# entn-at/tf-kaldi-speaker

Hardware: AMD Instinct MI355X
Metric: utterances/sec x-vector extraction (30-dim x 300-frame) (higher is better)
Workload: dtype f16+fp6-cross(f32-split); 1 GPU; tdnn x-vector (tdnn6_dense), statistics_pooling, 256 utt/GPU/step of 300 frames x 30 dims; batch_per_gpu=256, frames=300, node=tdnn6_dense, precision=f16f6, parallelism=utterance-shard x1, launch=stream launches

## Files before the change

### tf-kaldi-speaker_amd/csrc/gemm_f32.hip

```cpp
#include <mutex>

#include "xv_epilogue.h"

namespace xv {

constexpr int BM = 128, BN = 128, BK = 32;
constexpr int LDT = BK + 4;
constexpr int TILE_F = BM * LDT;

template <int FORM>
__global__ __launch_bounds__(256, 2) void gemm_f32_kernel(GemmArgs p, int nMt, int nNt, int kper) {
  extern __shared__ __attribute__((aligned(16))) float smem[];
  float* As = smem;
  float* Bs = smem + 2 * TILE_F;

  const int tid = threadIdx.x;
  const int lane = tid & 63, wave = tid >> 6;
  const int wm = wave >> 1, wn = wave & 1;
  const int r32 = lane & 31, h = lane >> 5;

  const int ntiles = nMt * nNt;
  const int slice = blockIdx.x / ntiles;
  const int tile = xcd_remap(blockIdx.x - slice * ntiles, ntiles);
  const int mt = tile / nNt, nt = tile - mt * nNt;
// ... 80 lines not shown
    for (int q = 0; q < BK / 8; ++q) {
      f32x4 a0 = *reinterpret_cast<const f32x4*>(ap + q * 8);
      f32x4 a1 = *reinterpret_cast<const f32x4*>(ap + 32 * LDT + q * 8);
      f32x4 b0 = *reinterpret_cast<const f32x4*>(bp + q * 8);
      f32x4 b1 = *reinterpret_cast<const f32x4*>(bp + 32 * LDT + q * 8);
#pragma unroll
      for (int j = 0; j < 4; ++j) {
        acc[0][0] = __builtin_amdgcn_mfma_f32_32x32x2f32(b0[j], a0[j], acc[0][0], 0, 0, 0);
        acc[0][1] = __builtin_amdgcn_mfma_f32_32x32x2f32(b0[j], a1[j], acc[0][1], 0, 0, 0);
        acc[1][0] = __builtin_amdgcn_mfma_f32_32x32x2f32(b1[j], a0[j], acc[1][0], 0, 0, 0);
        acc[1][1] = __builtin_amdgcn_mfma_f32_32x32x2f32(b1[j], a1[j], acc[1][1], 0, 0, 0);
      }
    }
    if (kt + 1 < nk) store_tiles(cur ^ 1);
    __syncthreads();
  }

  store_wave_tile(p, acc, m0 + wm * 64, n0 + wn * 64, lane, wave, reinterpret_cast<char*>(smem));
}

__global__ void splitk_reduce_kernel(GemmArgs p) {
  const int64_t total = (int64_t)p.M * p.N;
  for (int64_t i = (int64_t)blockIdx.x * blockDim.x + threadIdx.x; i < total; i += (int64_t)gridDim.x * blockDim.x) {
    const int m = (int)(i / p.N), n = (int)(i - (int64_t)m * p.N);
    float acc = 0.f;
    for (int s = 0; s < p.ksplit; ++s) acc += p.partial[((int64_t)s * p.M + m) * p.Npad + n];
    bool zero;
    const int orow = out_row(p, m, zero);
    if (orow < 0) continue;
    float v = fmaf(acc, p.scale[n], p.shift[n]);
    if (p.R) v += p.R[(int64_t)orow * p.ldr + n];
    p.Y[(int64_t)orow * p.ldy + n] = zero ? 0.f : apply_act(v, p.act, p.alpha ? p.alpha[n] : 0.f);
  }
}

int gemm_f32_ksplit(int M, int Kpad, int Npad) {
  if (M > 512) return 1;
  const int tiles = ((M + BM - 1) / BM) * (Npad / BN), nk = Kpad / BK;
  int s = 512 / (tiles > 0 ? tiles : 1);
  if (s > nk / 4) s = nk / 4;
  return s < 2 ? 1 : s;
}

hipError_t launch_gemm_f32(const GemmArgs& a, bool aligned, hipStream_t s) {
  if (a.M <= 0) return hipSuccess;
  const int nMt = (a.M + BM - 1) / BM, nNt = a.Npad / BN;
  const int ks = (a.ksplit > 1 && a.partial && !a.Ysb && !a.pool_part) ? a.ksplit : 1;
  const int nk_all = a.Kpad / BK;
  const int kper = (nk_all + ks - 1) / ks;
  const size_t smem = (size_t)4 * TILE_F * sizeof(float);
  static std::mutex init_mu;
  static bool attr_set[64] = {};
  int dev = 0;
  if (hipGetDevice(&dev) != hipSuccess) dev = 0;
  std::lock_guard<std::mutex> init_lock(init_mu);
  if (!attr_set[dev & 63]) {
    hipError_t e = hipFuncSetAttribute(reinterpret_cast<const void*>(gemm_f32_kernel<2>),
                                       hipFuncAttributeMaxDynamicSharedMemorySize, (int)smem);
    if (e != hipSuccess) return e;
    e = hipFuncSetAttribute(reinterpret_cast<const void*>(gemm_f32_kernel<1>),
                                       hipFuncAttributeMaxDynamicSharedMemorySize, (int)smem);
    if (e != hipSuccess) return e;
    e = hipFuncSetAttribute(reinterpret_cast<const void*>(gemm_f32_kernel<0>),
                            hipFuncAttributeMaxDynamicSharedMemorySize, (int)smem);
    if (e != hipSuccess) return e;
    attr_set[dev & 63] = true;
// ... 20 lines not shown
```

### tf-kaldi-speaker_amd/csrc/xv_kernels.h

```cpp
#pragma once
#include <hip/hip_runtime.h>
#include <stdint.h>

namespace xv {

enum Act : int { ACT_NONE = 0, ACT_RELU = 1, ACT_LRELU = 2, ACT_PRELU = 3, ACT_TANH = 4 };

constexpr float kLreluAlpha = 0.2f;
constexpr int kFlagWords = 8, kUttSmallWord = 4, kFeatMaxSlots = 32768;
constexpr float kVarFloor = 1e-12f;

struct GemmArgs {
  const float* X;
  int64_t ldx;
  int cin;
  int M;
  int K;
  int N;
  const float* Wt;
  int Kpad;
  int Npad;
  const float* scale;
  const float* shift;
  const float* alpha;
// ... 15 lines not shown
  int64_t bin_x_bytes = 0;
  float sb_mul = 1.f;
  int f16 = 0;
  long long* trace = nullptr;
  int ksplit;
  int raw;
  float* partial;
  int tail_mt = 0;
  float* pool_part;
  const int32_t* pool_row2utt;
  const int32_t* pool_slotbase;
  int64_t a_pitch;
  int64_t a_off;
  int64_t tap_stride;
  int ntaps;
  int ktap;
  const int32_t* arow;
  const float* R;
  int64_t ldr;
  const float* att_q = nullptr;
  float* att_part = nullptr;
  int64_t att_ld = 0;
  int att_heads = 0;
  const float* pool_w = nullptr;
  int pool_heads = 0;
  int pool_split = 0;
  int pool_dvh = 0;
  int pool_odim = 0;
};

hipError_t launch_gemm_f32(const GemmArgs& a, bool aligned, hipStream_t s);

int gemm_f32_ksplit(int M, int Kpad, int Npad);

int64_t gemm_bf16x3_tail_plan(int M, int Kpad, int Npad, int w, int* tail_mt, int* splits, int cb_quant = 1);

hipError_t launch_im2col_sb(const float* x, int64_t ldx, int cin, int w, int64_t rows, void* out_sb, int ldsb, int f16,
                            int* ovf, hipStream_t s);

hipError_t launch_gemm_bf16x3(const GemmArgs& a, hipStream_t s);
hipError_t launch_gemm_f16f6(const GemmArgs& a, hipStream_t s);
hipError_t launch_f6v2_tail_reduce(const GemmArgs& a, int nMain, hipStream_t s);
hipError_t launch_f6_from_sb(const void* sb, void* out, int64_t rows, int nblk, hipStream_t s);

hipError_t launch_build_rowmap(const int32_t* off0, int B, int ctx_in, int w, int32_t* rowmap, int M,
                               hipStream_t s);

hipError_t launch_stat_pool(const float* x, int64_t ldx, int C, const int32_t* off0, int B, int ctx,
                            float* out, int64_t ldo, hipStream_t s);

hipError_t launch_build_row2utt(const int32_t* off0, int B, int ctx, int32_t* row2utt, int M, hipStream_t s);
hipError_t launch_pool_finalize(const float* part, int C, const int32_t* off0, int B, int ctx,
                                const int32_t* slotbase, float* out, int64_t ldo, hipStream_t s);

hipError_t launch_build_rowmap_grid(const int32_t* off0, int B, int rows_per_t, int Fout, int So, int cover, int32_t* rowmap,
                                    int64_t M, hipStream_t s);
hipError_t launch_build_rowmap_grid_ts(const int32_t* off_in, const int32_t* off_out, int B, int rows_per_t, int Fout, int So,
                                       int ktime, int32_t* rowmap, int64_t M, hipStream_t s);
hipError_t launch_build_rowmap_grid_compact(const int32_t* off_in, const int32_t* off_out, int B, int Sin, int So, int Fout,
                                            int sw, int st, int ktime, int32_t* arow, int32_t* rowmap, int64_t M, int64_t Mpad,
                                            hipStream_t s);
hipError_t launch_grid_zero_border(const int32_t* off0, int B, int64_t frames, int F, int S, int chunks_y, int chunks_sb,
                                   float* y, void* ysb, hipStream_t s);
hipError_t launch_build_rowmap_rows(const int32_t* off0, int B, int32_t* rowmap, int64_t M, hipStream_t s);
hipError_t launch_build_rowmap_trows(const int32_t* off0, int B, int So, int32_t* rowmap, int64_t M, hipStream_t s);
hipError_t launch_build_rowmap_interior(const int32_t* off0, int B, int F, int S, int32_t* rowmap, int64_t M, hipStream_t s);
// ... 62 lines not shown
```

### tf-kaldi-speaker_amd/csrc/xvec_api.hip

```cpp
#include <hip/hip_runtime.h>

#include <algorithm>
#include <cmath>
#include <cstdarg>
#include <cstdio>
#include <cstring>
#include <map>
#include <mutex>
#include <string>
#include <vector>

#include "../../include/xvec_hip.h"
#include "xv_kernels.h"

using namespace xv;

namespace {

constexpr double kBnEps = 1e-3;
constexpr int kSlackRows = 512;
constexpr int kAlign = 256;

thread_local std::string g_last_error;

// ... 88 lines not shown

struct Op {
  int kind = OP_GEMM;
  int layer = -1;
  int in0 = -1, in1 = -1;
  int out = -1;
  int bnvec = -1;
};

struct Node {
  std::string name;
  int op = -1;
  int stage = -1;
  bool att_weights = false;
};

}

struct xv_handle {
  xv_model_desc desc{};
  int device = 0;
  bool finalized = false;
  std::string err;
  std::mutex mu;
  std::mutex err_mu;
  std::mutex prof_mu;
  int opt_pool_fusion = 1;
  int opt_tail_split = 1;
  int opt_onetap_f6_notail = 1;
  int opt_grid_f6 = 1;
  int opt_slab3 = 1;
  int opt_grid_compact = 1;
  int opt_att_fusion = 1;
  int opt_profile_dominant = 0;
  std::mutex pool_mu;
  std::vector<DevBuf> pool;
  size_t pool_bytes = 0;
  std::map<std::string, HostTensor> tensors;
  std::vector<Layer> layers;
  std::vector<Value> values;
  std::vector<Op> ops;
  std::vector<Node> nodes;
  DevBuf query;
  DevBuf ovf_flag;
  DevBuf query_eff;
  int key_npad = 0;
  int att_dk_h = 0, att_dk = 0, att_dv = 0;
  int final_ctx = 14;
  std::string post_bn_scope, post_alpha_name;
  DevBuf post_vec;
  int pool_dim = 0;
  struct ProfRec { hipEvent_t e0, e1; const xv_plan* plan; int step; };
  bool profiling = false;
  std::vector<hipEvent_t> prof_pool;
  size_t prof_next = 0;
  std::vector<ProfRec> prof_recs;
  int prof_forwards = 0;
};

struct PlanStep {
  int op = -1;
  int stage = -1;
  bool to_out = false;
  int64_t out_off = -1;
  int64_t out_sb_off = -1;
  int64_t in0_off = -1, in1_off = -1;
  int64_t in0_sb_off = -1;
  int64_t rows_in = 0, rows_out = 0;
  int M = 0;
  int rowmap = -1;
  int64_t scratch_off = -1;
  int64_t scratch2_off = -1;
  int ksplit = 1;
  int tail_mt = 0;
  bool fuse_pool = false;
  int lvl_in = 0, lvl_out = 0;
  int64_t frames_out = 0;
  bool grid_cover = false;
  bool out_f6 = false;
  bool trows = false;
  bool in_f6 = false;
  bool compact = false;
  int arow = -1;
  int fuse_att = 0;
  int64_t att_w_off = -1;
  int64_t att_s0_off = -1;
  int64_t att_ld = 0;
  bool unpad_to_out = false;
  int64_t flops = 0, bytes = 0;
};

struct xv_plan {
  xv_handle* h = nullptr;
  xv_plan_info info{};
  std::vector<int32_t> offsets;
  std::vector<int32_t> offsets_slotbase;
  DevBuf d_offsets;
  std::vector<int32_t> lvl_offsets[4];
  DevBuf d_lvl[4];
  const int32_t* dev_offsets(int level) const {
    return static_cast<const int32_t*>(level > 0 ? d_lvl[level].p : d_offsets.p);
  }
  DevBuf d_rowmaps;
  std::vector<int64_t> rowmap_off;
  std::vector<PlanStep> steps;
  DevBuf d_row2utt;
  DevBuf d_slotbase;
  int64_t pool_slots = 0;
  bool uniform_len = true;
  int uniform_L = 0;
  int dominant_step = 0;
};

namespace {

int fail(xv_handle* h, int code, const char* fmt, ...) {
  char buf[512];
  va_list ap;
  va_start(ap, fmt);
  vsnprintf(buf, sizeof(buf), fmt, ap);
  va_end(ap);
  if (h) {
    std::lock_guard<std::mutex> lk(h->err_mu);
    h->err = buf;
  }
  g_last_error = buf;
  return code;
}

#define XV_HIP(h, expr)                                                                              \
  do {                                                                                               \
    hipError_t _e = (expr);                                                                          \
    if (_e != hipSuccess)                                                                            \
      return fail((h), XV_ERR_HIP, "%s failed: %s (%s:%d)", #expr, hipGetErrorString(_e), __FILE__,  \
                  __LINE__);                                                                         \
  } while (0)

int64_t align_up(int64_t v, int64_t a) { return (v + a - 1) / a * a; }

constexpr size_t kPoolMaxBuffers = 96, kPoolMaxBytes = (size_t)1 << 30;
// ... 735 lines not shown
    }
    if (h->desc.att_apply_nonlinear) {
      const int n = h->pool_dim;
      std::vector<double> s, t;
      bn_fold(h, h->post_bn_scope, n, s, t);
      std::vector<float> vec((size_t)3 * n, 0.f);
      for (int i = 0; i < n; ++i) { vec[i] = (float)s[i]; vec[(size_t)n + i] = (float)t[i]; }
      if (!h->post_alpha_name.empty()) {
        const auto& a = T(h, h->post_alpha_name).data;
        for (int i = 0; i < n; ++i) vec[(size_t)2 * n + i] = a[i];
      }
      XV_HIP(h, h->post_vec.alloc(vec.size() * sizeof(float)));
      XV_HIP(h, hipMemcpy(h->post_vec.p, vec.data(), vec.size() * sizeof(float), hipMemcpyHostToDevice));
    }
  }
  XV_HIP(h, h->ovf_flag.alloc((kFlagWords + kFeatMaxSlots) * sizeof(int)));
  XV_HIP(h, hipMemset(h->ovf_flag.p, 0, (kFlagWords + kFeatMaxSlots) * sizeof(int)));
  XV_HIP(h, hipDeviceSynchronize());
  for (auto& kv : h->tensors) { kv.second.data.clear(); kv.second.data.shrink_to_fit(); }
  h->finalized = true;
  return XV_OK;
}

int xv_set_option(xv_handle* h, const char* name, int value) {
  if (!h || !name) return fail(h, XV_ERR_INVALID, "xv_set_option: null argument");
  std::lock_guard<std::mutex> lk(h->mu);
  if (!strcmp(name, "pool_fusion")) h->opt_pool_fusion = value != 0;
  else if (!strcmp(name, "tail_split")) h->opt_tail_split = value != 0;
  else if (!strcmp(name, "att_fusion")) h->opt_att_fusion = value != 0;
  else if (!strcmp(name, "slab3")) h->opt_slab3 = value != 0;
  else if (!strcmp(name, "onetap_f6_notail")) h->opt_onetap_f6_notail = value != 0;
  else if (!strcmp(name, "grid_f6")) h->opt_grid_f6 = value != 0;
  else if (!strcmp(name, "grid_compact")) h->opt_grid_compact = value != 0;
  else if (!strcmp(name, "profile_dominant")) h->opt_profile_dominant = value != 0;
  else return fail(h, XV_ERR_INVALID, "xv_set_option: unknown option '%s'", name);
  return XV_OK;
}

int xv_check_overflow(xv_handle* h, int reset) {
  if (!h) return fail(nullptr, XV_ERR_INVALID, "xv_check_overflow: null handle");
  if (!h->finalized || !h->ovf_flag.p) return 0;
  DeviceGuard g(h->device);
  std::vector<int32_t> w((size_t)kFlagWords + kFeatMaxSlots);
  XV_HIP(h, hipMemcpy(w.data(), h->ovf_flag.p, w.size() * sizeof(int32_t), hipMemcpyDeviceToHost));
  int32_t v[2] = {w[0], w[1]};
  for (int i = 0; i < kFeatMaxSlots; ++i) v[1] = std::max(v[1], w[(size_t)kFlagWords + i]);
  if (w[kUttSmallWord]) v[1] = w[kUttSmallWord];
  if (reset) XV_HIP(h, hipMemset(h->ovf_flag.p, 0, w.size() * sizeof(int32_t)));
  return xv_flags_decode(v);
}

int xv_flags_decode(const int32_t* flags) {
  if (!flags) return XV_ERR_INVALID;
  if (flags[0]) return 1;
  if (flags[1] > 0) {
    float mx;
    memcpy(&mx, &flags[1], 4);
    if (mx < 0.00390625f) return 2;
  }
  return 0;
}

int xv_flags_async(xv_handle* h, int32_t* host_flags, void* stream) {
  if (!h || !host_flags) return fail(h, XV_ERR_INVALID, "xv_flags_async: null argument");
  if (!h->finalized || !h->ovf_flag.p) { host_flags[0] = host_flags[1] = 0; return XV_OK; }
  DeviceGuard g(h->device);
// ... 150 lines not shown
  auto arena_free = [&](int64_t off, int64_t size) {
    free_list.push_back({off, size});
    std::sort(free_list.begin(), free_list.end(), [](const Block& a, const Block& b) { return a.off < b.off; });
    for (size_t i = 0; i + 1 < free_list.size();)
      if (free_list[i].off + free_list[i].size == free_list[i + 1].off) {
        free_list[i].size += free_list[i + 1].size;
        free_list.erase(free_list.begin() + i + 1);
      } else {
        ++i;
      }
  };

  std::vector<char> want_f32(h->values.size(), 0), want_sb(h->values.size(), 0);
  for (int o : order) {
    const Op& op = h->ops[o];
    const bool split_in = op.kind == OP_GEMM && h->layers[op.layer].use_split;
    if (op.in0 > 0) (split_in ? want_sb : want_f32)[op.in0] = 1;
    if (op.in1 > 0) want_f32[op.in1] = 1;
  }
  std::vector<int64_t> voff_sb(h->values.size(), -1), vsize_sb(h->values.size(), 0);

  int fused_value = -1;
  for (int o : order) {
    const Op& op = h->ops[o];
    if (op.kind != OP_STAT_POOL || op.in0 <= 0 || producer[op.in0] < 0) continue;
    const Op& prod = h->ops[producer[op.in0]];
    if (prod.kind != OP_GEMM || producer[op.in0] == node.op) continue;
    const Layer& L = h->layers[prod.layer];
    int readers = 0;
    for (int o2 : order)
      if (h->ops[o2].in0 == op.in0 || h->ops[o2].in1 == op.in0) ++readers;
    if (readers == 1 && L.w == 1 && (L.cout & 3) == 0 && h->opt_pool_fusion) fused_value = op.in0;
  }
  const int slot_value = fused_value >= 0 ? fused_value : att_pool_value;
  if (slot_value >= 0) {
    const int ctx = h->values[slot_value].ctx;
    const std::vector<int32_t>& so = lvl[h->values[slot_value].tlevel];
    std::vector<int32_t> slotbase(batch);
    int64_t nslots = 0;
    for (int b = 0; b < batch; ++b) {
      const int r0 = so[b] - b * ctx, r1 = so[b + 1] - (b + 1) * ctx;
      const int t0 = r0 >> 6, t1 = (r1 - 1) >> 6;
      slotbase[b] = (int32_t)(nslots - t0);
      nslots += t1 - t0 + 1;
    }
    p->pool_slots = nslots;
    p->offsets_slotbase = std::move(slotbase);
  }

  int64_t total_flops = 0;
  int64_t rowmap_elems = 0;
  for (size_t s = 0; s < order.size(); ++s) {
    const Op& op = h->ops[order[s]];
    PlanStep st;
    int64_t step_scratch = 0, step_scratch2 = 0;
    st.op = order[s];
    st.to_out = (order[s] == node.op);
    st.rows_in = op.in0 >= 0 ? value_rows(h, op.in0, Fl, batch) : 0;
    st.rows_out = value_rows(h, op.out, Fl, batch);
    st.lvl_in = op.in0 >= 0 ? h->values[op.in0].tlevel : 0;
    st.lvl_out = h->values[op.out].tlevel;
    st.frames_out = Fl[st.lvl_out];
    st.in0_off = op.in0 == 0 ? -2 : (op.in0 > 0 ? voff[op.in0] : -1);
    st.in0_sb_off = op.in0 > 0 ? voff_sb[op.in0] : -1;
    st.in1_off = op.in1 > 0 ? voff[op.in1] : -1;
    if (op.kind == OP_GEMM) {
// ... 4 lines not shown
      else if (L.mode == 1 && L.use_f6) {
        st.trows = true;
        st.M = (int)padded_rows;
      }
      else if ((L.mode == 1 || L.mode == 2) && L.use_split && h->opt_grid_compact &&
               st.rows_in * (int64_t)sb_ld(L.cin) * 4 < ((int64_t)1 << 32)) {
        st.compact = true;
        st.M = (int)(Fl[st.lvl_out] * L.Fout);
      }
      else if (L.mode == 1 || L.mode == 2) st.M = (int)(padded_rows * (h->values[op.in0].grid_S / L.sw));
      else if (L.mode == 3) st.M = (int)padded_rows;
      else st.M = (int)(padded_rows * h->values[op.out].grid_S);
      if (st.compact || st.trows) st.grid_cover = false;
      else if (L.mode == 1 || L.mode == 2) st.grid_cover = L.st == 1 && h->values[op.in0].grid_S / L.sw == h->values[op.out].grid_S;
      else if (L.mode == 4) st.grid_cover = true;
      if (L.w > 1 || L.mode != 0) {
        st.rowmap = (int)p->rowmap_off.size();
        p->rowmap_off.push_back(rowmap_elems);
        rowmap_elems += align_up(st.M, 64);
        if (st.compact) {
          st.arow = (int)p->rowmap_off.size();
          p->rowmap_off.push_back(rowmap_elems);
          rowmap_elems += align_up(st.M, 128);
        }
      }
      const int64_t valid_out = L.mode == 0 ? st.rows_out : Fl[st.lvl_out] * (L.mode == 3 ? 1 : L.Fout);
      st.flops = 2 * valid_out * (int64_t)L.cout * L.K();
      st.bytes = 4 * (st.rows_in * L.cin + st.rows_out * L.cout + (int64_t)L.K() * L.cout);
      int64_t scratch = 0;
      if (L.mode == 4) {
        scratch = ((int64_t)st.M + kSlackRows) * 32 * 4;
      } else if (L.im2col) {
        scratch = L.cin_pad ? (st.rows_in + kSlackRows) * (int64_t)L.cin_pad * 4 : (st.M + kSlackRows) * (int64_t)L.Kpad * 4;
      } else if (!L.use_split && op.out != fused_value) {
        st.ksplit = gemm_f32_ksplit(st.M, L.Kpad, L.Npad);
        if (st.ksplit > 1) scratch = (int64_t)st.ksplit * st.M * L.Npad * 4;
      } else if (L.use_f6) {
        scratch = (st.rows_in + kSlackRows) * (int64_t)sb_ld(L.cin) * 4;
        if (h->opt_tail_split && op.in1 <= 0 && L.mode == 0) {
          const int64_t part = gemm_bf16x3_tail_plan(st.M, L.Kpad, L.Npad, L.w, &st.tail_mt, &st.ksplit, 4);
          if (part > 0) {
            step_scratch2 = align_up(part, kAlign);
            st.scratch2_off = arena_alloc(step_scratch2);
          }
        }
      } else if (L.use_split && L.mode == 0 && op.out != fused_value && op.in1 <= 0 && h->opt_tail_split &&
                 order[s] != key_prod && order[s] != val_prod) {
        scratch = gemm_bf16x3_tail_plan(st.M, L.Kpad, L.Npad, L.w, &st.tail_mt, &st.ksplit);
      }
      if (scratch > 0) {
        step_scratch = align_up(scratch, kAlign);
        st.scratch_off = arena_alloc(step_scratch);
      }
    } else if (op.kind == OP_AFFINE_ACT) {
      st.stage = st.to_out ? node.stage : 2;
      st.bytes = 8 * st.rows_out * h->values[op.out].cols;
    } else if (op.kind == OP_ATT_POOL && val_prod >= 0) {
      st.fuse_att = 1;
      st.bytes = 4 * (p->pool_slots * (2 * (h->pool_dim / 2) + h->desc.att_num_heads) + st.rows_out * h->values[op.out].cols);
      st.flops = 8 * p->pool_slots * (h->pool_dim / 2);
    } else if (op.kind == OP_STAT_POOL || op.kind == OP_ATT_POOL) {
      st.bytes = 4 * (st.rows_in * h->values[op.in0].cols + st.rows_out * h->values[op.out].cols);
      st.flops = 4 * st.rows_in * h->values[op.in0].cols;
      if (op.kind == OP_STAT_POOL && op.in0 == fused_value) {
        st.fuse_pool = true;
        st.bytes = 4 * (p->pool_slots * 2 * h->values[op.in0].cols + st.rows_out * h->values[op.out].cols);
        st.flops = 6 * p->pool_slots * h->values[op.in0].cols;
      }
    } else if (op.kind == OP_ATT_SCORES) {
      st.bytes = 4 * st.rows_in * h->values[op.in0].cols;
      st.flops = 2 * st.rows_in * (int64_t)h->att_dk_h * h->desc.att_num_heads;
      if (key_prod >= 0) {
        st.fuse_att = 1;
        st.att_ld = align_up(st.rows_in, 64);
        st.bytes = 4 * (st.att_ld * (h->key_npad / 32) + st.rows_in) * h->desc.att_num_heads;
      }
    } else {
      st.bytes = 8 * st.rows_out * h->values[op.out].cols;
    }
    total_flops += st.flops;
    if (op.kind == OP_ATT_SOFTMAX) {
      voff[op.out] = voff[op.in0];
      vsize[op.out] = vsize[op.in0];
      vsize[op.in0] = 0;
      st.out_off = voff[op.out];
      if (val_prod >= 0) {
        st.fuse_att = 1;
        st.att_s0_off = voff[op.out] + align_up(st.rows_out * (int64_t)h->desc.att_num_heads * 4, kAlign);
      }
    } else if (st.to_out && !node.att_weights && h->values[op.out].grid_F == 0) {
      st.out_off = -1;
    } else if (st.to_out && !node.att_weights) {
      st.unpad_to_out = true;
      vsize[op.out] = value_bytes(h, op.out, Fl, batch);
      voff[op.out] = arena_alloc(vsize[op.out]);
      st.out_off = voff[op.out];
    } else {
      if (op.kind == OP_GEMM && order[s] == key_prod) {
// ... 8 lines not shown
        st.fuse_att = 2;
        vsize[op.out] = align_up(p->pool_slots * 2 * (int64_t)(h->pool_dim / 2) * 4, kAlign);
        voff[op.out] = arena_alloc(vsize[op.out]);
        st.out_off = voff[op.out];
        st.bytes = 4 * (st.rows_in * h->layers[op.layer].cin + (int64_t)h->layers[op.layer].K() * h->layers[op.layer].cout +
                        st.rows_out * h->desc.att_num_heads) + vsize[op.out];
        for (const PlanStep& prev : p->steps)
          if (h->ops[prev.op].kind == OP_ATT_SOFTMAX) { st.att_w_off = prev.out_off; st.att_s0_off = prev.att_s0_off; }
      } else if (op.out == fused_value) {
        st.fuse_pool = true;
        vsize[op.out] = align_up(p->pool_slots * 2 * (int64_t)h->values[op.out].cols * 4, kAlign);
        voff[op.out] = arena_alloc(vsize[op.out]);
        st.out_off = voff[op.out];
      } else if (want_f32[op.out] || node.att_weights) {
        vsize[op.out] = value_bytes(h, op.out, Fl, batch);
        if (op.kind == OP_ATT_SCORES && val_prod >= 0)
          vsize[op.out] = align_up(st.rows_out * (int64_t)h->desc.att_num_heads * 4, kAlign) +
                          align_up(p->pool_slots * (int64_t)h->desc.att_num_heads * 4, kAlign) + kAlign;
        voff[op.out] = arena_alloc(vsize[op.out]);
        st.out_off = voff[op.out];
      }
      if (want_sb[op.out]) {
        vsize_sb[op.out] = value_sb_bytes(h, op.out, Fl, batch);
        voff_sb[op.out] = arena_alloc(vsize_sb[op.out]);
        st.out_sb_off = voff_sb[op.out];
      }
    }
    if (op.kind == OP_ATT_POOL && val_prod >= 0)
      for (const PlanStep& prev : p->steps)
        if (h->ops[prev.op].kind == OP_ATT_SOFTMAX) st.att_s0_off = prev.att_s0_off;
    p->steps.push_back(st);
    if (step_scratch > 0) arena_free(st.scratch_off, step_scratch);
    if (step_scratch2 > 0) arena_free(st.scratch2_off, step_scratch2);
    for (int in : {op.in0, op.in1})
      if (in > 0 && last_use[in] == (int)s) {
        if (vsize[in] > 0) { arena_free(voff[in], vsize[in]); vsize[in] = 0; }
        if (vsize_sb[in] > 0) { arena_free(voff_sb[in], vsize_sb[in]); vsize_sb[in] = 0; }
      }
  }

  for (size_t i = 0; i < p->steps.size(); ++i)
    if (p->steps[i].flops > p->steps[p->dominant_step].flops) p->dominant_step = (int)i;

  for (PlanStep& cs : p->steps) {
    const Op& cop = h->ops[cs.op];
    if (cop.kind != OP_GEMM || !h->layers[cop.layer].use_f6) continue;
    const bool grid = h->layers[cop.layer].mode == 1;
    if (cs.in_f6) continue;
    int readers = 0;
    bool all_f6 = true;
    PlanStep* prod = nullptr;
    for (PlanStep& os : p->steps) {
      const Op& o = h->ops[os.op];
      if (o.in0 == cop.in0 || (!grid && o.in1 == cop.in0)) {
        ++readers;
        if (o.kind != OP_GEMM || !h->layers[o.layer].use_f6 || o.in0 != cop.in0) all_f6 = false;
      }
      if (o.out == cop.in0) prod = &os;
    }
    if (!prod || !all_f6 || (grid && readers != 1)) continue;
    const Op& pop = h->ops[prod->op];
    if (pop.kind != OP_GEMM) continue;
    const Layer& PL = h->layers[pop.layer];
    if (prod->to_out || prod->out_sb_off < 0 || prod->stage != PL.final_stage()) continue;
    if (grid) {
      const bool gather = PL.mode == 1 && !PL.use_f6 && PL.use_split && prod->compact && prod->out_off < 0 && pop.in1 <= 0;
// ... 62 lines not shown
      const Layer& L = h->layers[op.layer];
      const int ctx_in = h->values[op.in0].ctx;
      const int32_t* doff = p->dev_offsets(st.lvl_in);
      int32_t* rm = static_cast<int32_t*>(p->d_rowmaps.p) + p->rowmap_off[st.rowmap];
      if (L.mode == 0) e = launch_build_rowmap(doff, batch, ctx_in, L.w, rm, st.M, s);
      else if (st.trows) e = launch_build_rowmap_trows(doff, batch, h->values[op.out].grid_S, rm, st.M, s);
      else if (st.compact)
        e = launch_build_rowmap_grid_compact(doff, p->dev_offsets(st.lvl_out), batch, h->values[op.in0].grid_S,
                                             h->values[op.out].grid_S, L.Fout, L.sw, L.st, L.mode == 1 ? 3 : 1,
                                             static_cast<int32_t*>(p->d_rowmaps.p) + p->rowmap_off[st.arow], rm, st.M,
                                             align_up(st.M, 128), s);
      else if ((L.mode == 1 || L.mode == 2) && L.st == 2)
        e = launch_build_rowmap_grid_ts(doff, p->dev_offsets(st.lvl_out), batch, h->values[op.in0].grid_S / L.sw, L.Fout,
                                        h->values[op.out].grid_S, L.mode == 1 ? 3 : 1, rm, st.M, s);
      else if (L.mode == 1 || L.mode == 2)
        e = launch_build_rowmap_grid(doff, batch, h->values[op.in0].grid_S / L.sw, L.Fout, h->values[op.out].grid_S,
                                     st.grid_cover ? 1 : 0, rm, st.M, s);
      else if (L.mode == 3) e = launch_build_rowmap_rows(doff, batch, rm, st.M, s);
      else e = launch_build_rowmap_interior(doff, batch, L.Fout, h->values[op.out].grid_S, rm, st.M, s);
      if (e != hipSuccess) return bail(e, "build_rowmap");
    }
  }
  if (slot_value >= 0) {
    const int ctx = h->values[slot_value].ctx;
    const int64_t rows = value_rows(h, slot_value, Fl, batch);
    if ((e = pool_take(h, (size_t)rows * 4, p->d_row2utt)) != hipSuccess) return bail(e, "hipMalloc(row2utt)");
    if ((e = pool_take(h, (size_t)batch * 4, p->d_slotbase)) != hipSuccess) return bail(e, "hipMalloc(slotbase)");
    if ((e = hipMemcpyAsync(p->d_slotbase.p, p->offsets_slotbase.data(), (size_t)batch * 4, hipMemcpyHostToDevice, s)) != hipSuccess)
      return bail(e, "hipMemcpyAsync(slotbase)");
    if ((e = launch_build_row2utt(p->dev_offsets(h->values[slot_value].tlevel), batch, ctx,
                                  static_cast<int32_t*>(p->d_row2utt.p), (int)rows, s)) != hipSuccess)
      return bail(e, "build_row2utt");
  }
  *out = p;
  return XV_OK;
}

int xv_plan_query(const xv_plan* p, xv_plan_info* info) {
  if (!p || !info) return XV_ERR_INVALID;
  *info = p->info;
  return XV_OK;
}

void xv_plan_destroy(xv_plan* p) {
  if (!p) return;
  {
    DeviceGuard g(p->h->device);
    pool_give(p->h, p->d_offsets);
    for (int k = 1; k < 4; ++k) pool_give(p->h, p->d_lvl[k]);
    pool_give(p->h, p->d_rowmaps);
    pool_give(p->h, p->d_row2utt);
    pool_give(p->h, p->d_slotbase);
  }
  delete p;
}

static const char* step_name(const xv_handle* h, const PlanStep& st) {
  const Op& op = h->ops[st.op];
  switch (op.kind) {
    case OP_GEMM: {
      const Layer& L = h->layers[op.layer];
      if (!L.ep[ST_AFFINE].empty()) return L.ep[ST_AFFINE].c_str();
      const size_t a = L.kernel_name.find('/'), b = L.kernel_name.rfind('/');
      static thread_local std::string tmp;
      tmp = (a != std::string::npos && b > a) ? L.kernel_name.substr(a + 1, b - a - 1) : L.kernel_name;
      return tmp.c_str();
    }
    case OP_STAT_POOL: return "stat_pool";
    case OP_ATT_SCORES: return "att_scores";
    case OP_ATT_SOFTMAX: return "att_softmax";
    case OP_ATT_POOL: return "att_pool";
    case OP_AFFINE_ACT: return "att_post";
    case OP_L2_SCALE: return "l2_scale";
    case OP_GRID_MAXPOOL: return "conv0_max";
    default: return "op";
  }
}

static int run_plan(xv_handle* h, const xv_plan* p, const float* feats, int feat_ld, float* out, int64_t out_cap,
                    void* workspace, int64_t ws_bytes, hipStream_t s) {
  if (!h || !p) return fail(h, XV_ERR_INVALID, "xv_forward: null handle/plan");
  if (p->h != h) return fail(h, XV_ERR_INVALID, "xv_forward: plan belongs to another handle");
  if (!feats || !out) return fail(h, XV_ERR_INVALID, "xv_forward: null feature/output pointer");
  if (feat_ld < h->desc.feat_dim) return fail(h, XV_ERR_INVALID, "xv_forward: feat_ld %d < feature_dim %d", feat_ld, h->desc.feat_dim);
  if (out_cap < p->info.out_rows * p->info.out_cols)
// ... 190 lines not shown
            a.bin_x_bytes = (int64_t)L.cin * 4;
            if (a.Ysb) a.Ysb = static_cast<char*>(a.Ysb) + (int64_t)a.ldsb * 4;
            if (a.Y) a.Y += a.ldy;
            if (a.R) a.R += a.ldr;
          }
          if (st.tail_mt > 0 && st.scratch2_off >= 0) {
            a.tail_mt = st.tail_mt;
            a.ksplit = st.ksplit;
            a.partial = reinterpret_cast<float*>(ws + st.scratch2_off);
          }
          XV_HIP(h, launch_gemm_f16f6(a, s));
          if (st.unpad_to_out)
            XV_HIP(h, launch_grid_unpad_n(reinterpret_cast<const float*>(ws + st.out_off), off_out, B, vo.grid_F, vo.grid_S, vo.cols,
                                          st.frames_out, out, s));
          break;
        }
        if (L.use_split) {
          if (st.in0_sb_off < 0) return fail(h, XV_ERR_STATE, "split layer %s has no split-blocked input", L.kernel_name.c_str());
          a.Xsb = ws + st.in0_sb_off;
          a.ldsbx = L.mode == 0 ? sb_ld(L.cin) : 0;
          a.Wsb = L.wsb.p; a.Wfr = L.wfr.p;
          a.ysb_f6 = st.out_f6 ? 1 : 0;
          if (st.tail_mt > 0 && st.scratch_off >= 0) {
            a.tail_mt = st.tail_mt;
            a.ksplit = st.ksplit;
            a.partial = reinterpret_cast<float*>(ws + st.scratch_off);
          }
          XV_HIP(h, launch_gemm_bf16x3(a, s));
          if (st.unpad_to_out)
            XV_HIP(h, launch_grid_unpad_n(reinterpret_cast<const float*>(ws + st.out_off), off_out, B, vo.grid_F, vo.grid_S, vo.cols,
                                          st.frames_out, out, s));
          break;
        }
        if (st.ksplit > 1 && st.scratch_off >= 0) {
          a.ksplit = st.ksplit;
          a.partial = reinterpret_cast<float*>(ws + st.scratch_off);
        }
        const bool aligned = op.in0 != 0 && (a.ldx % 4 == 0) && (a.K % 4 == 0);
        if (L.mode != 0 && !aligned)
          return fail(h, XV_ERR_UNSUPPORTED, "resnet convolution %s needs channel counts that are multiples of 4", L.kernel_name.c_str());
        XV_HIP(h, launch_gemm_f32(a, aligned, s));
        if (st.unpad_to_out)
          XV_HIP(h, launch_grid_unpad_n(reinterpret_cast<const float*>(ws + st.out_off), off_out, B, vo.grid_F, vo.grid_S, vo.cols,
                                        st.frames_out, out, s));
        break;
      }
      case OP_STAT_POOL: {
        const Value& vi = h->values[op.in0];
        if (st.fuse_pool) {
          XV_HIP(h, launch_pool_finalize(in_ptr(st.in0_off), vi.cols, off_in, B, vi.ctx,
                                         static_cast<const int32_t*>(p->d_slotbase.p), optr, 2 * vi.cols, s));
          break;
        }
        XV_HIP(h, launch_stat_pool(in_ptr(st.in0_off), vi.cols, vi.cols, off_in, B, vi.ctx, optr, 2 * vi.cols, s));
        break;
      }
      case OP_ATT_SCORES: {
        const Value& vi = h->values[op.in0];
        const float scale = d.att_use_scale ? 1.0f / std::sqrt((float)h->att_dk_h) : 1.0f;
        if (st.fuse_att) {
          XV_HIP(h, launch_att_scores_reduce(in_ptr(st.in0_off), st.att_ld, h->key_npad / 32, d.att_num_heads, st.rows_in,
                                             scale, reinterpret_cast<float*>(ws + st.out_off), s));
          break;
        }
        XV_HIP(h, launch_att_scores(in_ptr(st.in0_off), vi.cols, st.rows_in, static_cast<const float*>(h->query.p),
                                    d.att_num_heads, h->att_dk_h, d.att_split_key, scale,
                                    reinterpret_cast<float*>(ws + st.out_off), s));
        break;
      }
      case OP_ATT_SOFTMAX: {
        float* sc = reinterpret_cast<float*>(ws + st.out_off);
        XV_HIP(h, launch_att_softmax(sc, d.att_num_heads, off, B, h->final_ctx, s));
        if (st.fuse_att)
          XV_HIP(h, launch_att_slot_sums(sc, d.att_num_heads, off, B, h->final_ctx, static_cast<const int32_t*>(p->d_slotbase.p),
                                         reinterpret_cast<float*>(ws + st.att_s0_off), s));
        if (st.to_out) XV_HIP(h, launch_att_weights_out(sc, d.att_num_heads, off, B, h->final_ctx, out, s));
        break;
      }
      case OP_ATT_POOL: {
        const Value& vv = h->values[op.in0];
        if (st.fuse_att) {
// ... 13 lines not shown
        const int a = st.stage >= 2 ? act_of(d) : ACT_NONE;
        XV_HIP(h, launch_affine_act(in_ptr(st.in0_off), n, B, n, vec, vec + n,
                                    (a == ACT_PRELU) ? vec + 2 * n : nullptr, a, optr, n, s));
        break;
      }
      case OP_GRID_MAXPOOL: {
        const Value& vo = h->values[op.out];
        float* y = st.out_off >= 0 ? reinterpret_cast<float*>(ws + st.out_off) : nullptr;
        XV_HIP(h, launch_grid_maxpool3x3(in_ptr(st.in0_off), off, B, vo.grid_F, vo.grid_S, vo.cols, st.rows_out, y,
                                         st.out_sb_off >= 0 ? ws + st.out_sb_off : nullptr, sb_ld(vo.cols), f16,
                                         static_cast<int*>(h->ovf_flag.p), std::ldexp(1.f, vo.sb_exp), s));
        if (st.unpad_to_out)
          XV_HIP(h, launch_grid_unpad_n(y, off_out, B, vo.grid_F, vo.grid_S, vo.cols, st.frames_out, out, s));
        break;
      }
      case OP_L2_SCALE: {
        XV_HIP(h, launch_l2_scale(in_ptr(st.in0_off), B, h->values[op.out].cols, d.feature_scaling_factor, optr, s));
        break;
      }
      default:
        return fail(h, XV_ERR_STATE, "unknown op kind %d", op.kind);
    }
    if (prof_step) {
      XV_HIP(h, hipEventRecord(pe1, s));
      std::lock_guard<std::mutex> lk(h->prof_mu);
      h->prof_recs.push_back({pe0, pe1, p, (int)si});
    }
  }
  return XV_OK;
}

int xv_forward(xv_handle* h, const xv_plan* p, const float* feats_dev, int feat_ld, float* out_dev, int64_t out_capacity,
               void* workspace, int64_t workspace_bytes, void* stream) {
  return run_plan(h, p, feats_dev, feat_ld, out_dev, out_capacity, workspace, workspace_bytes,
                  static_cast<hipStream_t>(stream));
}

int xv_profile_begin(xv_handle* h, int max_events) {
  if (!h) return fail(nullptr, XV_ERR_INVALID, "xv_profile_begin: null handle");
  if (max_events < 2) return fail(h, XV_ERR_INVALID, "xv_profile_begin: max_events < 2");
  DeviceGuard g(h->device);
  std::lock_guard<std::mutex> lk(h->prof_mu);
  while ((int)h->prof_pool.size() < max_events) {
    hipEvent_t e;
    XV_HIP(h, hipEventCreate(&e));
    h->prof_pool.push_back(e);
  }
  h->prof_next = 0;
  h->prof_recs.clear();
  h->prof_forwards = 0;
  h->profiling = true;
  return XV_OK;
}

int xv_profile_end(xv_handle* h, xv_kernel_time* entries, int max_entries, int* n_forwards) {
  if (!h) return fail(nullptr, XV_ERR_INVALID, "xv_profile_end: null handle");
  if (!h->profiling) return fail(h, XV_ERR_STATE, "xv_profile_end without xv_profile_begin");
  if (!entries || max_entries < 1) return fail(h, XV_ERR_INVALID, "xv_profile_end: no entry buffer");
  DeviceGuard g(h->device);
  std::lock_guard<std::mutex> lk(h->prof_mu);
  h->profiling = false;
  int n = 0;
  std::vector<int> count;
  for (const auto& r : h->prof_recs) {
    XV_HIP(h, hipEventSynchronize(r.e1));
    float ms = 0.f;
    XV_HIP(h, hipEventElapsedTime(&ms, r.e0, r.e1));
    const PlanStep& st = r.plan->steps[r.step];
// ... 161 lines not shown
```

Baseline: 225,200 utterances/s.

## Fuse statistics-pool finalize into head GEMM with split-K ticket reduction

```diff
diff --git a/tf-kaldi-speaker_amd/csrc/gemm_f32.hip b/tf-kaldi-speaker_amd/csrc/gemm_f32.hip
--- a/tf-kaldi-speaker_amd/csrc/gemm_f32.hip
+++ b/tf-kaldi-speaker_amd/csrc/gemm_f32.hip
@@ -136,6 +136,215 @@
     if (p.R) v += p.R[(int64_t)orow * p.ldr + n];
     p.Y[(int64_t)orow * p.ldy + n] = zero ? 0.f : apply_act(v, p.act, p.alpha ? p.alpha[n] : 0.f);
   }
+}
+
+constexpr int HBM = 32, HBN = 256;
+constexpr int H_TILE_A = HBM * LDT, H_TILE_B = HBN * LDT;
+constexpr int H_STAGE = H_TILE_A + H_TILE_B;
+constexpr int kHeadFastSlots = 8;
+
+__global__ __launch_bounds__(256, 1) void head_gemm_kernel(GemmArgs p, HeadArgs q, int nNt, int S, int kper) {
+  extern __shared__ __attribute__((aligned(16))) float smem[];
+  const int tid = threadIdx.x;
+  const int lane = tid & 63, wave = tid >> 6;
+  const int r32 = lane & 31, h = lane >> 5;
+  const int groups = S * nNt;
+  const int mt = blockIdx.x / groups, g = blockIdx.x - mt * groups;
+  const int slice = g / nNt, nt = g - slice * nNt;
+  const int tile = mt * nNt + nt;
+  const int m0 = mt * HBM, n0 = nt * HBN;
+  const int nk_all = p.Kpad / BK;
+  const int kt0 = slice * kper, nk = min(nk_all, kt0 + kper);
+
+  const int c4 = tid & 7, lr = tid >> 3;
+  const int b = m0 + lr;
+  const bool row_ok = b < p.M;
+  int r0 = 0, r1 = 1, t0 = 0, ns = 0;
+  int64_t base = 0;
+  if (row_ok) {
+    r0 = q.off0[b] - b * q.ctx;
+    r1 = q.off0[b + 1] - (b + 1) * q.ctx;
+    t0 = r0 >> 6;
+    ns = ((r1 - 1) >> 6) - t0 + 1;
+    base = (int64_t)q.slotbase[b] + t0;
+  }
+  const float len = (float)(r1 - r0);
+  const bool fast = ns <= kHeadFastSlots;
+  const int C = q.C;
+
+  f32x4 rb[8], s_i[kHeadFastSlots], q_i[kHeadFastSlots];
+  auto load_raw = [&](int kt) {
+    const int k = kt * BK + c4 * 4;
+#pragma unroll
+    for (int i = 0; i < 8; ++i) rb[i] = *reinterpret_cast<const f32x4*>(p.Wt + (int64_t)(n0 + lr + 32 * i) * p.Kpad + k);
+    if (!row_ok || !fast || k >= 2 * C) return;
+    const bool sd = k >= C;
+    const float* pp = q.part + (base * 2) * C + (sd ? k - C : k);
+#pragma unroll
+    for (int i = 0; i < kHeadFastSlots; ++i)
+      if (i < ns) {
+        s_i[i] = *reinterpret_cast<const f32x4*>(pp + (int64_t)i * 2 * C);
+        if (sd) q_i[i] = *reinterpret_cast<const f32x4*>(pp + ((int64_t)i * 2 + 1) * C);
+      }
+  };
+  auto finalize = [&](int kt) -> f32x4 {
+    const int k = kt * BK + c4 * 4;
+    f32x4 z = {0.f, 0.f, 0.f, 0.f};
+    if (!row_ok || k >= 2 * C) return z;
+    const bool sd = k >= C;
+    f32x4 s = z, m2 = z;
+    if (fast) {
+#pragma unroll
+      for (int i = 0; i < kHeadFastSlots; ++i)
+        if (i < ns) s += s_i[i];
+      const f32x4 mean = s / len;
+      if (!sd) return mean;
+#pragma unroll
+      for (int i = 0; i < kHeadFastSlots; ++i)
+        if (i < ns) {
+          const int t = t0 + i;
+          const int ni = min(r1, (t + 1) << 6) - max(r0, t << 6);
+          const f32x4 d = s_i[i] / (float)ni - mean;
+          m2 += q_i[i] + (float)ni * d * d;
+        }
+    } else {
+      const float* pp = q.part + (base * 2) * C + (sd ? k - C : k);
+      for (int i = 0; i < ns; ++i) s += *reinterpret_cast<const f32x4*>(pp + (int64_t)i * 2 * C);
+      const f32x4 mean = s / len;
+      if (!sd) return mean;
+      for (int i = 0; i < ns; ++i) {
+        const int t = t0 + i;
+        const int ni = min(r1, (t + 1) << 6) - max(r0, t << 6);
+        const f32x4 d = *reinterpret_cast<const f32x4*>(pp + (int64_t)i * 2 * C) / (float)ni - mean;
+        m2 += *reinterpret_cast<const f32x4*>(pp + ((int64_t)i * 2 + 1) * C) + (float)ni * d * d;
+      }
+    }
+    f32x4 var = m2 / len;
+#pragma unroll
+    for (int e = 0; e < 4; ++e) var[e] = sqrtf(var[e] <= kVarFloor ? kVarFloor : var[e]);
+    return var;
+  };
+  auto store_tiles = [&](int buf, f32x4 a) {
+    float* As = smem + buf * H_STAGE;
+    float* Bs = As + H_TILE_A;
+    *reinterpret_cast<f32x4*>(As + lr * LDT + c4 * 4) = a;
+#pragma unroll
+    for (int i = 0; i < 8; ++i) *reinterpret_cast<f32x4*>(Bs + (lr + 32 * i) * LDT + c4 * 4) = rb[i];
+  };
+
+  f32x16 acc[2];
+#pragma unroll
+  for (int i = 0; i < 2; ++i)
+#pragma unroll
+    for (int e = 0; e < 16; ++e) acc[i][e] = 0.f;
+
+  if (kt0 < nk) {
+    load_raw(kt0);
+    store_tiles(0, finalize(kt0));
+  }
+  __syncthreads();
+  for (int kt = kt0; kt < nk; ++kt) {
+    const int cur = (kt - kt0) & 1;
+    if (kt + 1 < nk) load_raw(kt + 1);
+    const float* ap = smem + cur * H_STAGE + r32 * LDT + 4 * h;
+    const float* bp = smem + cur * H_STAGE + H_TILE_A + (wave * 64 + r32) * LDT + 4 * h;
+#pragma unroll
+    for (int qq = 0; qq < BK / 8; ++qq) {
+      const f32x4 a0 = *reinterpret_cast<const f32x4*>(ap + qq * 8);
+      const f32x4 b0 = *reinterpret_cast<const f32x4*>(bp + qq * 8);
+      const f32x4 b1 = *reinterpret_cast<const f32x4*>(bp + 32 * LDT + qq * 8);
+#pragma unroll
+      for (int j = 0; j < 4; ++j) {
+        acc[0] = __builtin_amdgcn_mfma_f32_32x32x2f32(b0[j], a0[j], acc[0], 0, 0, 0);
+        acc[1] = __builtin_amdgcn_mfma_f32_32x32x2f32(b1[j], a0[j], acc[1], 0, 0, 0);
+      }
+    }
+    if (kt + 1 < nk) store_tiles(cur ^ 1, finalize(kt + 1));
+    __syncthreads();
+  }
+
+  float* slab = q.slabs + ((int64_t)tile * S + slice) * (HBM * HBN);
+#pragma unroll
+  for (int ni = 0; ni < 2; ++ni)
+#pragma unroll
+    for (int gq = 0; gq < 4; ++gq)
+      *reinterpret_cast<f32x4*>(slab + r32 * HBN + wave * 64 + ni * 32 + gq * 8 + 4 * h) =
+          f32x4{acc[ni][4 * gq], acc[ni][4 * gq + 1], acc[ni][4 * gq + 2], acc[ni][4 * gq + 3]};
+  asm volatile("s_waitcnt vmcnt(0)" ::: "memory");
+  __syncthreads();
+  int* flag = reinterpret_cast<int*>(smem);
+  if (tid == 0) {
+    __builtin_amdgcn_fence(__ATOMIC_RELEASE, "agent");
+    asm volatile("s_waitcnt vmcnt(0)" ::: "memory");
+    const unsigned old = __hip_atomic_fetch_add(q.tickets + tile, 1u, __ATOMIC_RELAXED, __HIP_MEMORY_SCOPE_AGENT);
+    const int last = old == (unsigned)(S - 1);
+    if (last) {
+      __hip_atomic_store(q.tickets + tile, 0u, __ATOMIC_RELAXED, __HIP_MEMORY_SCOPE_AGENT);
+      __builtin_amdgcn_fence(__ATOMIC_ACQUIRE, "agent");
+      asm volatile("s_waitcnt vmcnt(0)" ::: "memory");
+    }
+    *flag = last;
+  }
+  __syncthreads();
+  if (!*flag) return;
+
+  const float* slab0 = q.slabs + (int64_t)tile * S * (HBM * HBN);
+#pragma unroll 2
+  for (int j = 0; j < HBM * HBN / 4 / 256; ++j) {
+    const int idx = tid + 256 * j;
+    f32x4 v = {0.f, 0.f, 0.f, 0.f};
+#pragma unroll 8
+    for (int s = 0; s < S; ++s) v += *reinterpret_cast<const f32x4*>(slab0 + (int64_t)s * (HBM * HBN) + idx * 4);
+    const int m = m0 + (idx >> 6), n = n0 + (idx & 63) * 4;
+    bool zero;
+    const int orow = out_row(p, m, zero);
+    if (orow < 0) continue;
+#pragma unroll
+    for (int e = 0; e < 4; ++e) {
+      if (n + e >= p.N) break;
+      float y = fmaf(v[e], p.scale[n + e], p.shift[n + e]);
+      if (p.R) y += p.R[(int64_t)orow * p.ldr + n + e];
+      p.Y[(int64_t)orow * p.ldy + n + e] = zero ? 0.f : apply_act(y, p.act, p.alpha ? p.alpha[n + e] : 0.f);
+    }
+  }
+}
+
+int64_t head_gemm_plan(int M, int Kpad, int Npad, int* slices, int* tiles) {
+  *slices = 0;
+  *tiles = 0;
+  if (M <= 0 || M > 512 || Npad % HBN != 0 || Kpad % BK != 0) return 0;
+  const int nt = ((M + HBM - 1) / HBM) * (Npad / HBN), nk = Kpad / BK;
+  int s = 256 / nt;
+  if (s > 32) s = 32;
+  if (s > nk / 2) s = nk / 2;
+  if (s < 1) s = 1;
+  const int kper = (nk + s - 1) / s;
+  s = (nk + kper - 1) / kper;
+  *slices = s;
+  *tiles = nt;
+  return (int64_t)nt * s * HBM * HBN * 4;
+}
+
+hipError_t launch_head_gemm(const GemmArgs& a, const HeadArgs& q, int slices, hipStream_t s) {
+  if (a.M <= 0) return hipSuccess;
+  const int nMt = (a.M + HBM - 1) / HBM, nNt = a.Npad / HBN;
+  const int nk = a.Kpad / BK, kper = (nk + slices - 1) / slices;
+  const size_t smem = (size_t)2 * H_STAGE * sizeof(float);
+  static std::mutex init_mu;
+  static bool attr_set[64] = {};
+  int dev = 0;
+  if (hipGetDevice(&dev) != hipSuccess) dev = 0;
+  {
+    std::lock_guard<std::mutex> init_lock(init_mu);
+    if (!attr_set[dev & 63]) {
+      hipError_t e = hipFuncSetAttribute(reinterpret_cast<const void*>(head_gemm_kernel),
+                                         hipFuncAttributeMaxDynamicSharedMemorySize, (int)smem);
+      if (e != hipSuccess) return e;
+      attr_set[dev & 63] = true;
+    }
+  }
+  hipLaunchKernelGGL(head_gemm_kernel, dim3(nMt * nNt * slices), dim3(256), smem, s, a, q, nNt, slices, kper);
+  return hipGetLastError();
 }
 
 int gemm_f32_ksplit(int M, int Kpad, int Npad) {
diff --git a/tf-kaldi-speaker_amd/csrc/xv_kernels.h b/tf-kaldi-speaker_amd/csrc/xv_kernels.h
--- a/tf-kaldi-speaker_amd/csrc/xv_kernels.h
+++ b/tf-kaldi-speaker_amd/csrc/xv_kernels.h
@@ -71,6 +71,18 @@
 hipError_t launch_gemm_f32(const GemmArgs& a, bool aligned, hipStream_t s);
 
 int gemm_f32_ksplit(int M, int Kpad, int Npad);
+
+struct HeadArgs {
+  const float* part;
+  int C;
+  const int32_t* off0;
+  int ctx;
+  const int32_t* slotbase;
+  float* slabs;
+  unsigned* tickets;
+};
+int64_t head_gemm_plan(int M, int Kpad, int Npad, int* slices, int* tiles);
+hipError_t launch_head_gemm(const GemmArgs& a, const HeadArgs& q, int slices, hipStream_t s);
 
 int64_t gemm_bf16x3_tail_plan(int M, int Kpad, int Npad, int w, int* tail_mt, int* splits, int cb_quant = 1);
 
diff --git a/tf-kaldi-speaker_amd/csrc/xvec_api.hip b/tf-kaldi-speaker_amd/csrc/xvec_api.hip
--- a/tf-kaldi-speaker_amd/csrc/xvec_api.hip
+++ b/tf-kaldi-speaker_amd/csrc/xvec_api.hip
@@ -144,6 +144,7 @@
   int opt_slab3 = 1;
   int opt_grid_compact = 1;
   int opt_att_fusion = 1;
+  int opt_head_fusion = 1;
   int opt_profile_dominant = 0;
   std::mutex pool_mu;
   std::vector<DevBuf> pool;
@@ -198,6 +199,11 @@
   int64_t att_w_off = -1;
   int64_t att_s0_off = -1;
   int64_t att_ld = 0;
+  bool head = false;
+  bool head_skip = false;
+  int64_t head_part_off = -1;
+  int head_C = 0, head_ctx = 0, head_lvl = 0;
+  int head_slices = 0;
   bool unpad_to_out = false;
   int64_t flops = 0, bytes = 0;
 };
@@ -218,6 +224,8 @@
   std::vector<PlanStep> steps;
   DevBuf d_row2utt;
   DevBuf d_slotbase;
+  DevBuf d_tickets;
+  size_t ticket_bytes = 0;
   int64_t pool_slots = 0;
   bool uniform_len = true;
   int uniform_L = 0;
@@ -1019,6 +1027,7 @@
   else if (!strcmp(name, "onetap_f6_notail")) h->opt_onetap_f6_notail = value != 0;
   else if (!strcmp(name, "grid_f6")) h->opt_grid_f6 = value != 0;
   else if (!strcmp(name, "grid_compact")) h->opt_grid_compact = value != 0;
+  else if (!strcmp(name, "head_fusion")) h->opt_head_fusion = value != 0;
   else if (!strcmp(name, "profile_dominant")) h->opt_profile_dominant = value != 0;
   else return fail(h, XV_ERR_INVALID, "xv_set_option: unknown option '%s'", name);
   return XV_OK;
@@ -1235,6 +1244,28 @@
       if (h->ops[o2].in0 == op.in0 || h->ops[o2].in1 == op.in0) ++readers;
     if (readers == 1 && L.w == 1 && (L.cout & 3) == 0 && h->opt_pool_fusion) fused_value = op.in0;
   }
+  int head_pool_op = -1, head_gemm_op = -1;
+  if (h->opt_head_fusion && fused_value >= 0) {
+    const int C = h->values[fused_value].cols;
+    for (int o : order) {
+      const Op& op = h->ops[o];
+      if (op.kind != OP_STAT_POOL || op.in0 != fused_value || o == node.op || readers_of(op.out) != 1) continue;
+      for (int o2 : order) {
+        const Op& g = h->ops[o2];
+        if (g.kind != OP_GEMM || g.in0 != op.out || g.in1 > 0) continue;
+        const Layer& L = h->layers[g.layer];
+        int sl = 0, nt = 0;
+        if (!L.use_split && !L.im2col && L.mode == 0 && L.w == 1 && L.cin == 2 * C && (C & 3) == 0 &&
+            head_gemm_plan(batch, L.Kpad, L.Npad, &sl, &nt) > 0) {
+          head_pool_op = o;
+          head_gemm_op = o2;
+        }
+      }
+    }
+    if (head_gemm_op >= 0)
+      last_use[fused_value] = (int)(std::find(order.begin(), order.end(), head_gemm_op) - order.begin());
+  }
+  int head_tiles = 0;
   const int slot_value = fused_value >= 0 ? fused_value : att_pool_value;
   if (slot_value >= 0) {
     const int ctx = h->values[slot_value].ctx;
@@ -1305,6 +1336,13 @@
         scratch = ((int64_t)st.M + kSlackRows) * 32 * 4;
       } else if (L.im2col) {
         scratch = L.cin_pad ? (st.rows_in + kSlackRows) * (int64_t)L.cin_pad * 4 : (st.M + kSlackRows) * (int64_t)L.Kpad * 4;
+      } else if (order[s] == head_gemm_op) {
+        st.head = true;
+        scratch = head_gemm_plan(st.M, L.Kpad, L.Npad, &st.head_slices, &head_tiles);
+        st.head_part_off = voff[fused_value];
+        st.head_C = h->values[fused_value].cols;
+        st.head_ctx = h->values[fused_value].ctx;
+        st.head_lvl = h->values[fused_value].tlevel;
       } else if (!L.use_split && op.out != fused_value) {
         st.ksplit = gemm_f32_ksplit(st.M, L.Kpad, L.Npad);
         if (st.ksplit > 1) scratch = (int64_t)st.ksplit * st.M * L.Npad * 4;
@@ -1337,6 +1375,7 @@
       st.flops = 4 * st.rows_in * h->values[op.in0].cols;
       if (op.kind == OP_STAT_POOL && op.in0 == fused_value) {
         st.fuse_pool = true;
+        st.head_skip = order[s] == head_pool_op;
         st.bytes = 4 * (p->pool_slots * 2 * h->values[op.in0].cols + st.rows_out * h->values[op.out].cols);
         st.flops = 6 * p->pool_slots * h->values[op.in0].cols;
       }
@@ -1411,6 +1450,7 @@
     p->steps.push_back(st);
     if (step_scratch > 0) arena_free(st.scratch_off, step_scratch);
     if (step_scratch2 > 0) arena_free(st.scratch2_off, step_scratch2);
+    if (st.head && vsize[fused_value] > 0) { arena_free(voff[fused_value], vsize[fused_value]); vsize[fused_value] = 0; }
     for (int in : {op.in0, op.in1})
       if (in > 0 && last_use[in] == (int)s) {
         if (vsize[in] > 0) { arena_free(voff[in], vsize[in]); vsize[in] = 0; }
@@ -1539,6 +1579,11 @@
                                   static_cast<int32_t*>(p->d_row2utt.p), (int)rows, s)) != hipSuccess)
       return bail(e, "build_row2utt");
   }
+  if (head_tiles > 0) {
+    p->ticket_bytes = (size_t)head_tiles * 4;
+    if ((e = pool_take(h, p->ticket_bytes, p->d_tickets)) != hipSuccess) return bail(e, "hipMalloc(tickets)");
+    if ((e = hipMemsetAsync(p->d_tickets.p, 0, p->ticket_bytes, s)) != hipSuccess) return bail(e, "hipMemsetAsync(tickets)");
+  }
   *out = p;
   return XV_OK;
 }
@@ -1558,6 +1603,7 @@
     pool_give(p->h, p->d_rowmaps);
     pool_give(p->h, p->d_row2utt);
     pool_give(p->h, p->d_slotbase);
+    pool_give(p->h, p->d_tickets);
   }
   delete p;
 }
@@ -1814,6 +1860,19 @@
                                           st.frames_out, out, s));
           break;
         }
+        if (st.head) {
+          if (st.scratch_off < 0 || st.head_part_off < 0 || !p->d_tickets.p) return fail(h, XV_ERR_STATE, "segment head has no scratch");
+          HeadArgs q{};
+          q.part = reinterpret_cast<const float*>(ws + st.head_part_off);
+          q.C = st.head_C;
+          q.off0 = p->dev_offsets(st.head_lvl);
+          q.ctx = st.head_ctx;
+          q.slotbase = static_cast<const int32_t*>(p->d_slotbase.p);
+          q.slabs = reinterpret_cast<float*>(ws + st.scratch_off);
+          q.tickets = static_cast<unsigned*>(p->d_tickets.p);
+          XV_HIP(h, launch_head_gemm(a, q, st.head_slices, s));
+          break;
+        }
         if (st.ksplit > 1 && st.scratch_off >= 0) {
           a.ksplit = st.ksplit;
           a.partial = reinterpret_cast<float*>(ws + st.scratch_off);
@@ -1829,6 +1888,7 @@
       }
       case OP_STAT_POOL: {
         const Value& vi = h->values[op.in0];
+        if (st.head_skip) break;
         if (st.fuse_pool) {
           XV_HIP(h, launch_pool_finalize(in_ptr(st.in0_off), vi.cols, off_in, B, vi.ctx,
                                          static_cast<const int32_t*>(p->d_slotbase.p), optr, 2 * vi.cols, s));
@@ -1908,8 +1968,13 @@
 
 int xv_forward(xv_handle* h, const xv_plan* p, const float* feats_dev, int feat_ld, float* out_dev, int64_t out_capacity,
                void* workspace, int64_t workspace_bytes, void* stream) {
-  return run_plan(h, p, feats_dev, feat_ld, out_dev, out_capacity, workspace, workspace_bytes,
-                  static_cast<hipStream_t>(stream));
+  const int rc = run_plan(h, p, feats_dev, feat_ld, out_dev, out_capacity, workspace, workspace_bytes,
+                          static_cast<hipStream_t>(stream));
+  if (rc != XV_OK && h && p && p->h == h && p->d_tickets.p) {
+    DeviceGuard g(h->device);
+    (void)hipMemsetAsync(p->d_tickets.p, 0, p->ticket_bytes, static_cast<hipStream_t>(stream));
+  }
+  return rc;
 }
 
 int xv_profile_begin(xv_handle* h, int max_events) {
```

Result: slower. 222,100 utterances/s (-1.3%).
